# emilk/field_interpolation

Measured on AMD Instinct MI355X. Metric: solved lattice points/sec (assembly+CG to field within 1e-5 of the CPU reference by the solver's estimate: ended at rel. residual 1.1e-08), higher is better.
Workload: dtype f64

## Files before the change

field_interpolation_amd/csrc/fi_assembly.hip:

```cpp

#include "fi_prim.h"

#include "fi_internal.h"
#include "fi_rows.h"
#include "fi_sort.h"
#include "fi_nearest.h"

namespace fi {

namespace {

constexpr int kThreads = 256;

__host__ __device__ inline int packed_index(int i, int j, int nc)
{
	return i * nc - (i * (i - 1)) / 2 + (j - i);
}

template <int NC>
__device__ inline double block_row_sum(const double* B, int q)
{
	double s = 0.0;
#pragma unroll
	for (int j = 0; j < NC; ++j) { s += B[q <= j ? packed_index(q, j, NC) : packed_index(j, q, NC)]; }
// ... 806 lines not shown
		rhs  = c->pending[0]->rhs.as<float>();
	} else {
		key_cat.alloc(sizeof(uint32_t) * total);
		coef_cat.alloc(sizeof(float) * total * NC);
		rhs_cat.alloc(sizeof(float) * total);
		long at = 0;
		for (auto* pb : c->pending) {
			if (pb->nrows == 0) { continue; }
			FI_HIP_TRY(hipMemcpyAsync(key_cat.as<uint32_t>() + at, pb->key.p, sizeof(uint32_t) * pb->nrows,
			                          hipMemcpyDeviceToDevice, st));
			FI_HIP_TRY(hipMemcpyAsync(coef_cat.as<float>() + at * NC, pb->coef.p, sizeof(float) * pb->nrows * NC,
			                          hipMemcpyDeviceToDevice, st));
			FI_HIP_TRY(hipMemcpyAsync(rhs_cat.as<float>() + at, pb->rhs.p, sizeof(float) * pb->nrows,
			                          hipMemcpyDeviceToDevice, st));
			at += pb->nrows;
		}
		key  = key_cat.as<uint32_t>();
		coef = coef_cat.as<float>();
		rhs  = rhs_cat.as<float>();
	}

	DevBuf &row_in = c->scratch[3], &row_sorted = c->scratch[4], &key_sorted = c->scratch[5], &uniq = c->scratch[6],
	       &counts = c->scratch[7], &starts = c->scratch[8], &nruns = c->scratch[9], &tmp = c->scratch[10];
	row_in.alloc(sizeof(uint32_t) * total);
	row_sorted.alloc(sizeof(uint32_t) * total);
	key_sorted.alloc(sizeof(uint32_t) * total);
	uniq.alloc(sizeof(uint32_t) * total);
	counts.alloc(sizeof(uint32_t) * total);
	starts.alloc(sizeof(uint32_t) * total);
	nruns.alloc(sizeof(uint32_t) * 4);
	hipLaunchKernelGGL(k_iota, dim3(blocks_for(total)), dim3(kThreads), 0, st, row_in.as<uint32_t>(), total);
	int end_bit = 1;
	while ((1ull << end_bit) <= invalid) { ++end_bit; }
	size_t tb = 0;
	FI_HIP_TRY(sort_pairs_u32(nullptr, tb, key, key_sorted.as<uint32_t>(), row_in.as<uint32_t>(), row_sorted.as<uint32_t>(),
	                          static_cast<unsigned int>(total), 0, end_bit, st));
	tmp.alloc(tb);
	FI_HIP_TRY(sort_pairs_u32(tmp.p, tb, key, key_sorted.as<uint32_t>(), row_in.as<uint32_t>(), row_sorted.as<uint32_t>(),
	                          static_cast<unsigned int>(total), 0, end_bit, st));
	size_t tb2 = 0;
	FI_HIP_TRY(prim::run_length_encode(nullptr, tb2, key_sorted.as<uint32_t>(), uniq.as<uint32_t>(), counts.as<uint32_t>(),
	                                    nruns.as<uint32_t>(), static_cast<size_t>(total), st));
	DevBuf& tmp2 = c->scratch[11];
	tmp2.alloc(tb2);
	FI_HIP_TRY(prim::run_length_encode(tmp2.p, tb2, key_sorted.as<uint32_t>(), uniq.as<uint32_t>(), counts.as<uint32_t>(),
	                                    nruns.as<uint32_t>(), static_cast<size_t>(total), st));
	DevBuf& tail3 = c->scratch[26];
	tail3.alloc(sizeof(uint32_t) * 3);
	DevBuf& heavy = c->scratch[28];
	heavy.alloc(sizeof(uint32_t) * (static_cast<size_t>(total / kHeavyRows) + 2));
	hipLaunchKernelGGL(k_rle_tail, dim3(1), dim3(1), 0, st, nruns.as<uint32_t>(), uniq.as<uint32_t>(), counts.as<uint32_t>(),
	                   tail3.as<uint32_t>(), heavy.as<uint32_t>());
	uint32_t* h_tail = static_cast<uint32_t*>(pinned(c, 0, 3 * sizeof(uint32_t)));
	FI_HIP_TRY(hipMemcpyAsync(h_tail, tail3.p, 3 * sizeof(uint32_t), hipMemcpyDeviceToHost, st));
// ... 332 lines not shown
```

field_interpolation_amd/csrc/fi_capi.hip:

```cpp
#include "fi_solver_internal.h"
#include "fi_workers.h"
#include "fi_iso.h"
#include "fi_dual.h"
#include "fi_sample.h"
#include "fi_nearest.h"
#include "fi_knn.h"
#include "fi_orient.h"
#include "fi_surface.h"
#include "fi_ray.h"
#include "fi_robust.h"
#include "fi_parts.h"
#include "fi_simplify.h"
#include "fi_smooth.h"
#include "fi_meshpts.h"

#include <memory>

namespace fi {

static thread_local std::string g_error;

void set_error(const char* fmt, ...)
{
	char    buf[1024];
// ... 432 lines not shown
namespace fi {
void finish_assemble_timing(fi_ctx* c)
{
	if (!c->asm_time_pending) { return; }
	c->asm_time_pending = false;
	if (hipEventSynchronize(c->ev_asm1) != hipSuccess) { return; }
	float ms = 0;
	if (hipEventElapsedTime(&ms, c->ev_asm0, c->ev_asm1) == hipSuccess) { c->stats.assemble_ms = ms; }
}
}

int fi_assemble(fi_ctx* c)
{
	FI_API_BEGIN
	fi::check_ctx(c);
	fi::bind_device(c);
	fi::finish_assemble_timing(c);
	if (!c->ev_asm0) {
		FI_HIP_TRY(hipEventCreate(&c->ev_asm0));
		FI_HIP_TRY(hipEventCreate(&c->ev_asm1));
	}
	const hipEvent_t e0 = c->ev_asm0, e1 = c->ev_asm1;
	fi::chain_mark(nullptr);
	FI_HIP_TRY(hipEventRecord(e0, c->stream));
	{
		bool trip = c->generic.ntrip != 0, grad = !fi::holds_value_rows_only(c);
		if (c->facts_forced) {
			trip = c->forced_trip;
			grad = c->forced_grad;
		} else if (c->nranks > 1 && fi::comm_ready(c)) {
			double* slot = (c->scal.as<fi::CgScalars>() + 2)->sums;
			double  v[2] = {trip ? 1.0 : 0.0, grad ? 1.0 : 0.0};
			FI_HIP_TRY(hipMemcpyAsync(slot, v, sizeof(v), hipMemcpyHostToDevice, c->stream));
			fi::allreduce_sum(c, slot, 2);
			FI_HIP_TRY(hipMemcpyAsync(v, slot, sizeof(v), hipMemcpyDeviceToHost, c->stream));
			FI_HIP_TRY(hipStreamSynchronize(c->stream));
			trip = v[0] > 0.0;
			grad = v[1] > 0.0;
		}
		c->any_trip        = trip;
		c->value_rows_only = !grad && !trip;
		c->facts_forced    = false;
	}
	const int reach = fi::model_reach(c->w);
	const int want_reach = reach > 1 ? reach : 1;
	int want_halo = want_reach;
// ... 81 lines not shown
		};
		fi::Worker *helper = nullptr, *helper2 = nullptr;
		try {
			if (!lumped) {
				helper = fi::worker_pool().acquire();
				helper->run(build);
			}
			if (mixed64) {
				helper2 = fi::worker_pool().acquire();
				helper2->run(build2);
			}
		} catch (...) {
		}
		int main_code = FI_OK;
		c->defer_scaling_exchange = true;
		try {
			fi::AllocStream alloc_on(c->stream);
			fi::chain_mark("threads started");
			fi::assemble(c);
			fi::chain_mark("finest: rows assembled");
			fi::generic_assemble(c);
			fi::stencil_prepare(c);
			fi::chain_mark("finest: stencil prepared");
			fi::operator_prepare(c);
			fi::chain_mark("finest: operator prepared");
		} catch (const fi::Fail& f) {
			main_code = f.code;
		} catch (...) {
			main_code = FI_ERR_HIP;
			fi::set_error("unexpected exception while assembling the finest level");
		}
		if (lumped && main_code == FI_OK) {
			try {
				fi::AllocStream alloc_on(c->stream);
				c->twin->defer_scaling_exchange = true;
				fi::twin_assemble_lumped(c);
				fi::chain_mark("finest: lumped replica");
			} catch (const fi::Fail& f) {
				main_code = f.code;
			} catch (...) {
				main_code = FI_ERR_HIP;
				fi::set_error("unexpected exception while building the lumped replica");
			}
		}
		if (helper) {
			helper->wait();
			fi::worker_pool().release(helper);
// ... 359 lines not shown
{
	FI_API_BEGIN
	fi::check_assembled(c);
	fi::bind_device(c);
	FI_REQUIRE(x && y, FI_ERR_INVALID, "null vector");
	c->dtype == FI_F64 ? fi::apply_f64_t<double>(c, x, y) : fi::apply_f64_t<float>(c, x, y);
	FI_API_END
}

int fi_get_Atb_f64(fi_ctx* c, double* out)
{
	FI_API_BEGIN
	fi::check_assembled(c);
	fi::bind_device(c);
	c->dtype == FI_F64 ? fi::get_vec_f64_t<double>(c, c->atb, out) : fi::get_vec_f64_t<float>(c, c->atb, out);
	FI_API_END
}

int fi_get_diag_f64(fi_ctx* c, double* out)
{
	FI_API_BEGIN
	fi::check_assembled(c);
	fi::bind_device(c);
	c->dtype == FI_F64 ? fi::get_vec_f64_t<double>(c, c->diag, out) : fi::get_vec_f64_t<float>(c, c->diag, out);
	FI_API_END
}

int fi_get_stats(const fi_ctx* c, fi_stats* out)
{
	FI_API_BEGIN
	fi::check_ctx(c);
	FI_REQUIRE(out != nullptr, FI_ERR_INVALID, "null output");
	fi::finish_assemble_timing(const_cast<fi_ctx*>(c));
	*out = c->stats;
	out->coarse_unconverged = 0;
	const fi_ctx* top = c->twin && c->twin->coarse ? c->twin : c;
	for (const fi_ctx* l = top->coarse; l; l = l->coarse) {
		if (!l->unwatched_pending || !l->ev_unwatched || !l->pin[2]) { continue; }
		if (hipEventSynchronize(l->ev_unwatched) != hipSuccess) { continue; }
		const fi::CgScalars* was = static_cast<const fi::CgScalars*>(l->pin[2]);
		const bool met = was->done == 1 || was->done == 5 || was->done == 4;
		if (!met) { out->coarse_unconverged += 1; }
		out->coarse_iterations += (met ? was->iter : l->unwatched_expected) - l->unwatched_expected;
	}
	FI_API_END
}

int fi_time_apply(fi_ctx* c, int reps, double* ms_per_launch)
{
	FI_API_BEGIN
	fi::check_assembled(c);
	fi::bind_device(c);
	FI_REQUIRE(reps > 0 && ms_per_launch, FI_ERR_INVALID, "bad arguments");
	fi::ensure_vectors(c);
	fi::CgScalars init{};
	FI_HIP_TRY(hipMemcpyAsync(c->scal.p, &init, sizeof(init), hipMemcpyHostToDevice, c->stream));
	fi::EventPair timer;
	const hipEvent_t e0 = timer.e0, e1 = timer.e1;
	const char* which = fi::tuning_switch("FI_TIME_STEP");
	const int   step = which ? atoi(which) : 0;
	auto launch = [&]() {
		if (step >= 1 && fi::stencil_cheb_available(c)) {
			c->dtype == FI_F64 ? fi::ensure_poly_vectors<double>(c) : fi::ensure_poly_vectors<float>(c);
			if (step == 1) {
				fi::stencil_cheb_step(c, c->r.p, nullptr, c->r.p, c->mg_d.p, 0.3, 0.2, c->partial.as<double>(), 0, 0.0, 0.5);
			} else if (step == 2) {
				fi::stencil_cheb_step(c, c->mg_d.p, c->mg_x.p, c->r.p, c->mg_x.p, 0.3, 0.2, c->partial.as<double>(), 0, 0.5);
			} else {
				fi::stencil_cheb_step(c, c->mg_x.p, c->mg_d.p, c->r.p, c->mg_d.p, 0.3, 0.2, c->partial.as<double>());
			}
		} else {
			fi::apply_AtA(c, c->p.p, c->q.p, c->partial.as<double>());
		}
	};
	launch();
	FI_HIP_TRY(hipEventRecord(e0, c->stream));
	for (int k = 0; k < reps; ++k) { launch(); }
	FI_HIP_TRY(hipEventRecord(e1, c->stream));
	FI_HIP_TRY(hipEventSynchronize(e1));
	float ms = 0;
	FI_HIP_TRY(hipEventElapsedTime(&ms, e0, e1));
	*ms_per_launch = ms / reps;
	FI_API_END
// ... 584 lines not shown
```

field_interpolation_amd/csrc/fi_cg.hip:

```cpp
#include "fi_solver_internal.h"

namespace fi {

namespace {
struct PredKey {
	int    kind, dtype, ndim, gn[3], level, below, mixed, rows_only;
	float  w[8];
	double tol;
	bool operator<(const PredKey& o) const { return std::memcmp(this, &o, sizeof(PredKey)) < 0; }
};
PredKey pred_key(const fi_ctx* c, int kind, double tol)
{
	PredKey k;
	std::memset(&k, 0, sizeof(k));
	k.kind  = kind;
	k.dtype = c->dtype;
	k.ndim  = c->g.ndim;
	for (int d = 0; d < 3; ++d) { k.gn[d] = c->g.gn[d]; }
	k.level = c->level;
	for (const fi_ctx* l = (c->twin && c->twin->coarse ? c->twin->coarse : c->coarse); l; l = l->coarse) { ++k.below; }
	k.mixed     = c->mixed;
	k.rows_only = c->value_rows_only ? 1 : 0;
	const float w[8] = {c->w.data_pos, c->w.data_gradient, c->w.model_0, c->w.model_1, c->w.model_2, c->w.model_3, c->w.model_4,
	                    c->w.gradient_smoothness};
// ... 494 lines not shown
	double  v = mine ? 1.0 : 0.0;
	FI_HIP_TRY(hipMemcpyAsync(flag, &v, sizeof(double), hipMemcpyHostToDevice, c0->stream));
	allreduce_sum(c0, flag, 1);
	FI_HIP_TRY(hipMemcpyAsync(&v, flag, sizeof(double), hipMemcpyDeviceToHost, c0->stream));
	FI_HIP_TRY(hipStreamSynchronize(c0->stream));
	return v > 0.0;
}

bool all_ranks_ok(fi_ctx* c, bool mine)
{
	if (!(c->nranks > 1 && comm_ready(c))) { return mine; }
	double* flag = (c->scal.as<CgScalars>() + 2)->sums + 3;
	double  v = mine ? 0.0 : 1.0;
	FI_HIP_TRY(hipMemcpyAsync(flag, &v, sizeof(double), hipMemcpyHostToDevice, c->stream));
	allreduce_sum(c, flag, 1);
	FI_HIP_TRY(hipMemcpyAsync(&v, flag, sizeof(double), hipMemcpyDeviceToHost, c->stream));
	FI_HIP_TRY(hipStreamSynchronize(c->stream));
	return v == 0.0;
}

template <typename T>
void cg_run(RankSet& R, int max_iterations, float tol)
{
	fi_ctx* c0 = R[0];
	hipStream_t st = c0->stream;
	if (max_iterations <= 0) {
		const int64_t dflt = 2 * static_cast<int64_t>(c0->g.gn[0]) * c0->g.gn[1] * c0->g.gn[2];
		max_iterations = dflt > std::numeric_limits<int>::max() ? std::numeric_limits<int>::max() : static_cast<int>(dflt);
	}
	const double tolerance = tol > 0 ? static_cast<double>(tol) : static_cast<double>(std::numeric_limits<float>::epsilon());

	if (c0->unwatched_pending) {
		c0->unwatched_pending = false;
		FI_HIP_TRY(hipEventSynchronize(c0->ev_unwatched));
		const CgScalars* was = static_cast<const CgScalars*>(pinned(c0, 2, sizeof(CgScalars)));
		const bool as_expected = (was->done == 1 || was->done == 5) && was->iter > 0 && was->iter <= c0->unwatched_expected;
		c0->last_cg_iterations = as_expected ? was->iter : 0;
		c0->pred_recalled[0]   = true;
		c0->cg_count_recalled  = false;
	}
	if (c0->level > 0 && R.size() == 1 && c0->last_cg_iterations == 0) {
		const int n = recall_iterations(c0, 0, tolerance);
		if (n > 0) {
			c0->last_cg_iterations = n;
			c0->last_cg_tol        = tolerance;
			c0->cg_count_recalled  = true;
// ... 323 lines not shown
			FI_HIP_TRY(hipMemcpyAsync(g0.p, c->x.p, elem_size(c) * c->g.nloc, hipMemcpyDeviceToDevice, c->stream));
			kept[i] = &g0;
		}
	}
	cg_run<T>(R, 4000, sizeof(T) == 8 ? 1e-12f : 1e-6f);
	for (size_t i = 0; i < R.size(); ++i) {
		if (kept[i]) { generic_keep_guess_in_empty_tiles(R[i], tile_size, kept[i]->p, R[i]->x.p); }
	}
}

template <typename T>
void tile_pass_t(fi_ctx* c, const float* guess, int tile_size, float* out, int memory)
{
	ensure_vectors(c);
	load_owned<T>(c, c->x, guess, memory);
	RankSet R{c};
	tile_pass_run<T>(R, tile_size);
	store_owned<T>(c, c->x, out, memory);
}

template <typename T>
void jacobi_run(RankSet& R, int sweeps, float weight)
{
	CgScalars init{};
	reset_scalars(R, init);
	for (int s = 0; s < sweeps; ++s) {
		halo_exchange(R, &fi_ctx::x);
		for (fi_ctx* c : R) { apply_AtA(c, c->x.p, c->q.p, nullptr); }
		for (fi_ctx* c : R) {
			const int64_t o = c->g.own_first;
			hipLaunchKernelGGL((k_jacobi_update<T>), dim3(stream_blocks(c->g.nown)), dim3(kThreads), 0, c->stream, c->g.nown,
			                   static_cast<T>(weight), c->atb.as<T>() + o, c->q.as<T>() + o, c->dinv.as<T>() + o,
			                   c->x.as<T>() + o);
		}
	}
	FI_HIP_TRY(hipGetLastError());
}

template <typename T>
void jacobi_t(fi_ctx* c, const float* guess, int sweeps, float weight, float* out, int memory)
{
	ensure_vectors(c);
	load_owned<T>(c, c->x, guess, memory);
	RankSet R{c};
	jacobi_run<T>(R, sweeps, weight);
	store_owned<T>(c, c->x, out, memory);
// ... 114 lines not shown
```

field_interpolation_amd/csrc/fi_internal.h:

```cpp
#pragma once

#include <hip/hip_runtime.h>

#include <chrono>
#include <cstdint>
#include <cstdio>
#include <cstdlib>
#include <string>
#include <utility>
#include <vector>

#include "../../include/fi_hip.h"

namespace fi {

inline const char* test_switch(const char* name) { return getenv(name); }
#ifdef FI_TIMING_BUILD
inline const char* tuning_switch(const char* name) { return getenv(name); }
#else
inline const char* tuning_switch(const char*) { return nullptr; }
#endif

inline std::chrono::steady_clock::time_point& chain_origin()
{
// ... 307 lines not shown
	fi::DevBuf dinv16;
	fi::DevBuf dinv16s;
	bool       dinv16s_valid = false;
	bool       lumped = false;
	fi::DevBuf dlump;
	hipEvent_t ev_asm0 = nullptr, ev_asm1 = nullptr;
	bool       asm_time_pending = false;
	bool       want_lump = false;
	fi::DevBuf lump;
	bool       data_pinned = false;
	double     mg_safe = 4.0;
	int        mg_terms = 5;
	double     mg_pratio = 30.0;
	int        mg_cheb_degree = 0;
	double     mg_cheb_ratio = 0.0;
	int        mg_kcycle = 0;
	fi::DevBuf kc;
	int        mg_smoother = 1;
	bool       any_trip = false;
	bool       facts_forced = false, forced_trip = false, forced_grad = false;
	bool       value_rows_only = false;
	bool       scaling_ghosts = false;
	bool       defer_scaling_exchange = false;
	fi::DevBuf x, r, p, q;
	fi::DevBuf mg_b, mg_x, mg_r, mg_d;
	double     lambda_max = 0;
	int        poly_terms = 0;
	double     poly_ratio = 10.0;
	double     poly_lambda = 0;
	int        last_mg_iterations = 0;
	double     last_mg_tol = 0;
	bool       predictable_start = false;
	double     last_cg_tol = 0;
	bool       unwatched_pending = false;
	int        unwatched_expected = 0;
	hipEvent_t ev_unwatched = nullptr;
	int        last_cg_iterations = 0;
	double     field_tol = 0;
	bool       pred_recalled[2] = {false, false};
	bool       cg_count_recalled = false;
	int        last_outer_iterations = 0;
	int        mg_mode = 0;
	fi::DevBuf partial;
	fi::DevBuf scal;
	fi::CgScalars* scal_host = nullptr;
	void*      pin[3] = {nullptr, nullptr, nullptr};
	size_t     scal_host_cap = 0;
	size_t     pin_bytes[3] = {0, 0, 0};
	int        max_blocks = 0;

	fi::DevBuf scratch[36];

	bool       bx_dot_wanted = false, bx_dot_done = false;
	bool       tail_ok = false;
	fi::DevBuf tail_dia, tail_map, tail_prog;
	bool       tail_prog_valid = false;
	bool       dia_valid = false;
	int        tail_nlev = 0, tail_nops = 0;
	int        tail_lds_floats = 0;

	fi::Comm*  comm = nullptr;
	hipStream_t comm_stream = nullptr;
	hipStream_t level_stream = nullptr;
	hipEvent_t  ev_level = nullptr;
	hipStream_t level_stream2 = nullptr;
	hipStream_t build_stream = nullptr;
	hipEvent_t  ev_build = nullptr;
	hipEvent_t  ev_level2 = nullptr;
	hipEvent_t  ev_ready = nullptr, ev_halo = nullptr;
	fi::DevBuf group_scal;
	bool       owns_stream = true;
	bool       owns_comm = true;
	int        mixed = 0;
	fi_ctx*    twin = nullptr;
	int        tile_ts = 0;
	int        verify_residual = 1;
	fi_stats   stats{};
	std::vector<hipEvent_t> ev;
	std::vector<hipEvent_t> ev_prec;
	int        prec_budget = 0, prec_taken = 0, prec_chain_launches = 0;
	double     prec_chain_bytes = 0;
};

namespace fi {

size_t elem_size(const fi_ctx* c);

void operator_prepare(fi_ctx* c, bool with_scaling = false, const float* lump_in = nullptr);
void apply_AtA(fi_ctx* c, const void* x, void* y, double* pq_partial);
int  apply_num_partials(const fi_ctx* c);
double apply_algorithmic_bytes(const fi_ctx* c);
void error_map(fi_ctx* c, const void* x, void* out);
void exchange_halo(fi_ctx* c, void* v, int width = 0);
void exchange_halo_on(fi_ctx* c, void* v, hipStream_t stream, int width = 0);
bool comm_ready(const fi_ctx* c);
void operator_finish_ghosts(fi_ctx* c);
void operator_rescale_with_ghosts(fi_ctx* c);
void prepare_safe_scaling(fi_ctx* c);

void stencil_prepare(fi_ctx* c);
int  stencil_partials(const fi_ctx* c);
bool stencil_apply(fi_ctx* c, const void* x, void* y, double* partial);
bool stencil_apply_part(fi_ctx* c, const void* x, void* y, double* partial, int part);

bool cells_fused(const fi_ctx* c);
bool stencil_cheb_available(const fi_ctx* c);
int  stencil_cheb_partials(const fi_ctx* c);
void stencil_cheb_step(fi_ctx* c, const void* z, const void* zprev, const void* r, void* znew, double c1, double c2,
                       double* partial, int part = 0, double zprev_scale = 0.0, double pro_scale = 0.0,
                       const unsigned short* scaling = nullptr,
                       int extend = 0,
// ... 50 lines not shown
```

field_interpolation_amd/csrc/fi_levels.hip:

```cpp
#include "fi_solver_internal.h"
#include "fi_workers.h"

namespace fi {

int plan_levels(const fi_ctx* c, int* first_tail)
{
	const int D = c->g.ndim;
	int n[3] = {c->g.gn[0], c->g.gn[1], c->g.gn[2]};
	std::vector<int> lo(c->nranks), hi(c->nranks);
	for (int r = 0; r < c->nranks; ++r) {
		lo[r] = static_cast<int>(static_cast<int64_t>(r) * n[D - 1] / c->nranks);
		hi[r] = static_cast<int>(static_cast<int64_t>(r + 1) * n[D - 1] / c->nranks);
	}
	int levels = 0, tail = 0;
	const bool allow_tail = c->nranks > 1 && !test_switch("FI_NO_REPLICATED_TAIL");
	for (int l = 1; l <= c->levels_wanted; ++l) {
		bool ok = true;
		for (int d = 0; d < D; ++d) {
			n[d] = (n[d] + 1) / 2;
			ok = ok && n[d] >= 8;
		}
		if (!ok) { break; }
		if (c->nranks > 1 && !tail) {
			bool thick = true;
// ... 274 lines not shown
                                                           float* __restrict__ diag)
{
	for (int64_t i = static_cast<int64_t>(blockIdx.x) * kThreads + threadIdx.x; i < n; i += static_cast<int64_t>(gridDim.x) * kThreads) {
		const float v = sums[i];
		const float f = v > 0.0f ? v : 0.0f;
		dlump[i] = f;
		diag[i]  = f;
	}
}

void twin_assemble_lumped(fi_ctx* c)
{
	fi_ctx* t = c->twin;
	t->stream = c->stream;
	for (auto* pb : t->pending) { t->pending_pool.push_back(pb); }
	t->pending.clear();
	generic_clear(t);
	assemble(t);
	const Geom& g = c->g;
	FI_REQUIRE(c->want_lump && c->lump.p, FI_ERR_STATE, "the lumped replica needs the row sums of the fp64 level's assembly");
	generic_assemble(t);
	stencil_prepare(t);
	if (g.nown == g.nloc && t->nranks == 1 && g.nloc > (1 << 16)) {
		operator_prepare(t, true, c->lump.as<float>());
		return;
	}
	t->dlump.alloc(sizeof(float) * g.nloc);
	if (g.nown != g.nloc) { FI_HIP_TRY(hipMemsetAsync(t->dlump.p, 0, sizeof(float) * g.nloc, c->stream)); }
	hipLaunchKernelGGL(k_lumped_diag, dim3(stream_blocks(g.nown)), dim3(kThreads), 0, c->stream, g.nown,
	                   c->lump.as<float>() + g.own_first, t->dlump.as<float>() + g.own_first, t->diag.as<float>() + g.own_first);
	FI_HIP_TRY(hipGetLastError());
	operator_prepare(t, t->nranks == 1);
}

fi_ctx* twin_prepare(fi_ctx* c)
{
	if (c->level != 0) { return nullptr; }
	if (!(c->mixed && c->dtype == FI_F64)) {
		if (c->twin) {
			fi_ctx_destroy(c->twin);
			c->twin = nullptr;
		}
		return nullptr;
	}
	const int D = c->g.ndim;
	{
		long from_points = 0;
// ... 104 lines not shown
```

field_interpolation_amd/csrc/fi_multigrid.hip:

```cpp
#include "fi_solver_internal.h"

namespace fi {

template <typename T>
bool cascade_guess(RankSet& R, RankSet* wide)
{
	bool wrote_wide = false;
	std::vector<RankSet> chains;
	{
		RankSet cur = R;
		for (;;) {
			chains.push_back(cur);
			RankSet next;
			for (fi_ctx* c : cur) {
				if (c->coarse) { next.push_back(c->coarse); }
			}
			if (next.size() != cur.size()) { break; }
			cur = next;
		}
	}
	for (auto& lev : chains) {
		for (fi_ctx* c : lev) { ensure_vectors(c); }
	}
	for (fi_ctx* c : chains.back()) { FI_HIP_TRY(hipMemsetAsync(c->x.p, 0, sizeof(T) * c->g.nloc, c->stream)); }
// ... 437 lines not shown
		}
	} else if (Rfine[0]->nranks > 1) {
		allreduce_sum_vec(Rfine[0], (Rc[0]->*v).p, n, sizeof(T) == 8);
	}
}

RankSet coarse_of(const RankSet& R)
{
	RankSet r;
	for (fi_ctx* c : R) { r.push_back(c->coarse); }
	return r;
}

void apply_all(RankSet& R, Vec in, Vec out, bool partials)
{
	halo_exchange(R, in);
	for (fi_ctx* c : R) { apply_AtA(c, (c->*in).p, (c->*out).p, partials ? c->partial.as<double>() : nullptr); }
}


template <typename T>
void estimate_lambda(RankSet& R)
{
	for (fi_ctx* c : R) { mg_alloc<T>(c); }
	CgScalars init{};
	reset_scalars(R, init);
	auto nbv = [](fi_ctx* c) { return stream_blocks(c->g.nown); };
	for (fi_ctx* c : R) {
		hipLaunchKernelGGL((k_seed<T>), dim3(nbv(c)), dim3(kThreads), 0, c->stream, c->g.nown, global_first(c),
		                   vown<T>(c, &fi_ctx::mg_d));
	}
	const int steps = 10;
	double sums[2] = {0, 0};
	for (int k = 0; k < steps; ++k) {
		apply_all(R, &fi_ctx::mg_d, &fi_ctx::q, false);
		for (fi_ctx* c : R) {
			hipLaunchKernelGGL((k_power_step<T>), dim3(nbv(c)), dim3(kThreads), 0, c->stream, c->g.nown, vown<T>(c, &fi_ctx::q),
			                   vown<T>(c, &fi_ctx::dinv), vown<T>(c, &fi_ctx::mg_d), c->partial.as<double>());
		}
		if (k >= steps - 2) {
			reduce_phase(R, 1, nbv, nbv, -1);
			fi_ctx* c0 = R[0];
			FI_HIP_TRY(hipMemcpyAsync(c0->scal_host, c0->scal.p, sizeof(CgScalars), hipMemcpyDeviceToHost, c0->stream));
			FI_HIP_TRY(hipStreamSynchronize(c0->stream));
			sums[k - (steps - 2)] = c0->scal_host->sums[0];
		}
	}
	const double lambda = (sums[0] > 0 && sums[1] > 0) ? std::sqrt(sums[1] / sums[0]) : 2.0;
	for (fi_ctx* c : R) { c->lambda_max = lambda; }
}

bool smooth_fused_ok(const RankSet& R)
{
	if (test_switch("FI_NO_FUSED_SMOOTHER")) { return false; }
	for (const fi_ctx* c : R) {
		if (!stencil_full_epi_available(c)) { return false; }
	}
	return true;
}
void swap_vectors(RankSet& R, Vec a, Vec b)
{
	if (a == b) { return; }
	for (fi_ctx* c : R) {
		(c->*a).swap(c->*b);
	}
}
template <typename T>
void cheb_smooth_fused(RankSet& R, Vec b, Vec x, int degree, double ratio, bool from_zero)
{
	const double hi = 1.1 * R[0]->lambda_max, lo = hi / ratio;
	const double theta = 0.5 * (hi + lo), delta = 0.5 * (hi - lo), sigma = theta / delta;
	const Vec ring[3] = {x, &fi_ctx::mg_d, &fi_ctx::mg_r};
	int cur = 0, prev = -1;
	auto step = [&](double a, double c1, double c2) {
		const int next = prev < 0 ? (cur + 1) % 3 : 3 - cur - prev;
		halo_exchange(R, ring[cur]);
		for (fi_ctx* c : R) {
			stencil_full_step(c, (c->*ring[cur]).p, prev < 0 ? nullptr : (c->*ring[prev]).p, (c->*b).p, false,
			                  (c->*ring[next]).p, a, c1, c2);
		}
		prev = cur;
		cur  = next;
	};
	bool have_prev = false;
	if (from_zero) {
		for (fi_ctx* c : R) {
			hipLaunchKernelGGL((k_cheb_first16<T>), dim3(stream_blocks(c->g.nown)), dim3(kThreads), 0, c->stream, c->g.nown,
			                   vown<T>(c, b), c->dinv16.as<unsigned short>() + c->g.own_first, vown<T>(c, x),
			                   static_cast<T>(1.0 / theta));
		}
	} else {
		step(1.0, 0.0, 1.0 / theta);
		have_prev = true;
	}
	double rho = 1.0 / sigma;
	for (int k = 1; k < degree; ++k) {
		const double rho_new = 1.0 / (2.0 * sigma - rho);
		const double c1 = rho_new * rho, c2 = 2.0 * rho_new / delta;
		if (!have_prev) { prev = -1; }
		step(1.0 + c1, c1, c2);
		have_prev = true;
		rho = rho_new;
	}
	swap_vectors(R, x, ring[cur]);
}

template <typename T>
void cheb_smooth(RankSet& R, Vec b, Vec x, int degree, double ratio, bool from_zero)
{
	if (smooth_fused_ok(R)) {
		cheb_smooth_fused<T>(R, b, x, degree, ratio, from_zero);
		return;
	}
	const double hi = 1.1 * R[0]->lambda_max, lo = hi / ratio;
	const double theta = 0.5 * (hi + lo), delta = 0.5 * (hi - lo), sigma = theta / delta;
	auto nbv = [](fi_ctx* c) { return stream_blocks(c->g.nown); };
	if (from_zero) {
		for (fi_ctx* c : R) {
			hipLaunchKernelGGL((k_cheb_first<T>), dim3(nbv(c)), dim3(kThreads), 0, c->stream, c->g.nown, vown<T>(c, b),
			                   vown<T>(c, &fi_ctx::dinv), degree > 1 ? vown<T>(c, &fi_ctx::mg_d) : vown<T>(c, x),
			                   static_cast<T>(1.0 / theta));
		}
	} else {
		apply_all(R, x, &fi_ctx::q, false);
		for (fi_ctx* c : R) {
			hipLaunchKernelGGL((k_cheb_init<T>), dim3(nbv(c)), dim3(kThreads), 0, c->stream, c->g.nown, vown<T>(c, b),
			                   vown<T>(c, &fi_ctx::q), vown<T>(c, &fi_ctx::dinv), vown<T>(c, &fi_ctx::mg_r),
			                   vown<T>(c, &fi_ctx::mg_d), vown<T>(c, x), static_cast<T>(1.0 / theta), 0);
		}
	}
	double rho = 1.0 / sigma;
	for (int k = 1; k < degree; ++k) {
// ... 1173 lines not shown
```

field_interpolation_amd/csrc/fi_operator.hip:

```cpp

#include "fi_internal.h"

namespace fi {

namespace {

constexpr int kThreads = 256;

__device__ inline double wave_sum(double v)
{
	for (int o = 32; o > 0; o >>= 1) { v += __shfl_down(v, o, 64); }
	return v;
}

__device__ inline double block_sum(double v)
{
	__shared__ double s[kThreads / 64];
	v = wave_sum(v);
	const int lane = threadIdx.x & 63, wave = threadIdx.x >> 6;
	if (lane == 0) { s[wave] = v; }
	__syncthreads();
	double r = 0;
	if (threadIdx.x == 0) {
		for (int w = 0; w < kThreads / 64; ++w) { r += s[w]; }
// ... 411 lines not shown
	mc.on[5] = w.gradient_smoothness > 0.0f;
	mc.gs    = mc.on[5] ? static_cast<T>(w.gradient_smoothness) : T(0);
	return mc;
}

constexpr int kDiagRows = 4;
template <typename T>
__global__ __launch_bounds__(kThreads) void k_model_diag3(Geom g, ModelCoef<T> mc, T* __restrict__ diag, T* __restrict__ dinv,
                                                          unsigned short* __restrict__ d16, unsigned short* __restrict__ d16s, T factor,
                                                          const float* __restrict__ lump_in, float* __restrict__ dlump_out)
{
	const int ext0 = g.own_hi[0] - g.own_lo[0], ext1 = g.own_hi[1] - g.own_lo[1];
	const int x = static_cast<int>(blockIdx.x) * kThreads + threadIdx.x;
	if (x >= ext0) { return; }
	const int lx = g.own_lo[0] + x, lz = g.own_lo[2] + static_cast<int>(blockIdx.z);
	const int y0 = static_cast<int>(blockIdx.y) * kDiagRows;
	T in[kDiagRows];
#pragma unroll
	for (int j = 0; j < kDiagRows; ++j) {
		const int64_t idx = lx * g.stride[0] + (g.own_lo[1] + y0 + j) * g.stride[1] + lz * g.stride[2];
		if (lump_in) {
			const float v = y0 + j < ext1 ? lump_in[idx] : 0.0f;
			in[j] = static_cast<T>(v > 0.0f ? v : 0.0f);
			if (y0 + j < ext1) { dlump_out[idx] = static_cast<float>(in[j]); }
		} else {
			in[j] = y0 + j < ext1 ? diag[idx] : T(0);
		}
	}
#pragma unroll
	for (int j = 0; j < kDiagRows; ++j) {
		if (y0 + j >= ext1) { break; }
		const int ly = g.own_lo[1] + y0 + j;
		const int64_t idx = lx * g.stride[0] + ly * g.stride[1] + lz * g.stride[2];
		T acc = 0;
#pragma unroll
		for (int d = 0; d < 3; ++d) {
			const int li = d == 0 ? lx : (d == 1 ? ly : lz);
			const int c = li + g.off[d], n = g.gn[d];
			if (mc.on[0]) { acc += mc.w0sq; }
			for (int k = 1; k <= 4; ++k) {
				if (!mc.on[k]) { continue; }
				for (int m = 0; m <= k; ++m) {
					const int a = c - m;
					if (a >= 0 && a + k < n) { acc += mc.c[k][m] * mc.c[k][m]; }
				}
			}
		}
		const T d = in[j] + acc;
		__builtin_nontemporal_store(d, diag + idx);
		if (dinv) {
			const T v = (d != T(0)) ? T(1) / d : T(1);
			__builtin_nontemporal_store(v, dinv + idx);
			__builtin_nontemporal_store(static_cast<unsigned short>(__float_as_uint(static_cast<float>(v)) >> 16), d16 + idx);
		}
		if (d16s) {
			const T dd = d > acc ? d - acc : T(0);
			const T sc = acc + factor * dd;
			const T v  = (sc > T(0)) ? T(1) / sc : T(1);
			__builtin_nontemporal_store(static_cast<unsigned short>(__float_as_uint(static_cast<float>(v)) >> 16), d16s + idx);
		}
	}
}

template <int D, typename T>
void prepare_dim(fi_ctx* c, bool with_scaling, const float* lump_in)
{
	const Geom& g = c->g;
	const ModelCoef<T> mc = make_coef<T>(c->w);
	c->dinv.alloc(sizeof(T) * g.nloc);
	c->dinv16.alloc(sizeof(unsigned short) * g.nloc);
	const bool whole = g.nown == g.nloc;
	const int ext1 = g.own_hi[1] - g.own_lo[1], ext2 = g.own_hi[2] - g.own_lo[2];
	const bool fuse_scaling = with_scaling && whole && c->nranks == 1 && g.nloc > (1 << 16);
	FI_REQUIRE(!lump_in || (D == 3 && !mc.on[5] && ext1 <= 65535 && ext2 <= 65535 && whole && sizeof(T) == 4), FI_ERR_STATE,
	           "lumped replica: unexpected lattice");
	if (D == 3 && !mc.on[5] && ext1 <= 65535 && ext2 <= 65535) {
		if (fuse_scaling) { c->dinv16s.alloc(sizeof(unsigned short) * g.nloc); }
		if (lump_in) { c->dlump.alloc(sizeof(float) * g.nloc); }
		hipLaunchKernelGGL((k_model_diag3<T>), dim3((g.own_hi[0] - g.own_lo[0] + kThreads - 1) / kThreads, (ext1 + kDiagRows - 1) / kDiagRows, ext2),
		                   dim3(kThreads), 0, c->stream, g, mc, c->diag.as<T>(), whole ? c->dinv.as<T>() : static_cast<T*>(nullptr),
		                   whole ? c->dinv16.as<unsigned short>() : static_cast<unsigned short*>(nullptr),
		                   fuse_scaling ? c->dinv16s.as<unsigned short>() : static_cast<unsigned short*>(nullptr),
		                   static_cast<T>(c->lumped ? 1.0 : c->mg_safe), lump_in, lump_in ? c->dlump.as<float>() : static_cast<float*>(nullptr));
		if (fuse_scaling) {
			c->data_pinned   = false;
			c->dinv16s_valid = true;
		}
	} else
	hipLaunchKernelGGL((k_model_diag<D, T>), dim3(blocks_for(g.nown)), dim3(kThreads), 0, c->stream, g, mc,
	                   c->diag.as<T>(), whole ? c->dinv.as<T>() : static_cast<T*>(nullptr),
	                   whole ? c->dinv16.as<unsigned short>() : static_cast<unsigned short*>(nullptr));
	c->scaling_ghosts = false;
	if (!whole) {
		if (c->nranks > 1 && comm_ready(c) && !c->defer_scaling_exchange) {
			exchange_halo(c, c->diag.p, c->min_slab >= c->halo ? c->halo : c->reach);
			c->scaling_ghosts = true;
		}
		hipLaunchKernelGGL((k_invert_diag<T>), dim3(blocks_for(g.nloc)), dim3(kThreads), 0, c->stream, g.nloc,
		                   c->diag.as<T>(), c->dinv.as<T>(), c->dinv16.as<unsigned short>());
	}
	FI_HIP_TRY(hipGetLastError());
}

template <typename T>
void finish_ghosts_t(fi_ctx* c)
{
	const Geom& g = c->g;
	exchange_halo(c, c->diag.p, c->min_slab >= c->halo ? c->halo : c->reach);
	hipLaunchKernelGGL((k_invert_diag<T>), dim3(blocks_for(g.nloc)), dim3(kThreads), 0, c->stream, g.nloc, c->diag.as<T>(),
	                   c->dinv.as<T>(), c->dinv16.as<unsigned short>());
	FI_HIP_TRY(hipGetLastError());
	c->scaling_ghosts = true;
}

template <int D, typename T>
void safe_scaling_dim(fi_ctx* c)
{
	const Geom& g = c->g;
	const ModelCoef<T> mc = make_coef<T>(c->w);
	c->dinv16s.alloc(sizeof(unsigned short) * g.nloc);
	unsigned int* weak = nullptr;
	DevBuf cnt;
	if (g.nloc <= (1 << 16) && c->nranks == 1) {
		cnt.alloc(sizeof(unsigned int));
		FI_HIP_TRY(hipMemsetAsync(cnt.p, 0, sizeof(unsigned int), c->stream));
		weak = cnt.as<unsigned int>();
	}
	hipLaunchKernelGGL((k_safe_scaling<D, T>), dim3(blocks_for(g.nloc)), dim3(kThreads), 0, c->stream, g, mc, c->diag.as<T>(),
	                   static_cast<T>(c->lumped ? 1.0 : c->mg_safe), c->dinv16s.as<unsigned short>(), weak);
	FI_HIP_TRY(hipGetLastError());
	c->data_pinned = false;
	if (weak) {
		unsigned int* h = static_cast<unsigned int*>(pinned(c, 0, sizeof(unsigned int)));
		*h = 1;
		FI_HIP_TRY(hipMemcpyAsync(h, weak, sizeof(unsigned int), hipMemcpyDeviceToHost, c->stream));
		FI_HIP_TRY(hipStreamSynchronize(c->stream));
		c->data_pinned = *h == 0;
	}
	c->dinv16s_valid = true;
}

int cells_partials(const fi_ctx* c) { return capped_blocks(c->cells.ncell); }

template <int D, typename T>
void apply_dim(fi_ctx* c, const T* x, T* y, double* partial)
// ... 225 lines not shown
	c->defer_scaling_exchange = false;
	if (c->nranks <= 1 || !comm_ready(c) || c->g.nown == c->g.nloc) { return; }
	c->dtype == FI_F64 ? finish_ghosts_t<double>(c) : finish_ghosts_t<float>(c);
	c->dinv16s_valid = false;
}

void operator_rescale_with_ghosts(fi_ctx* c)
{
	const Geom& g = c->g;
	if (c->dtype == FI_F64) {
		hipLaunchKernelGGL((k_invert_diag<double>), dim3(blocks_for(g.nloc)), dim3(kThreads), 0, c->stream, g.nloc, c->diag.as<double>(),
		                   c->dinv.as<double>(), c->dinv16.as<unsigned short>());
	} else {
		hipLaunchKernelGGL((k_invert_diag<float>), dim3(blocks_for(g.nloc)), dim3(kThreads), 0, c->stream, g.nloc, c->diag.as<float>(),
		                   c->dinv.as<float>(), c->dinv16.as<unsigned short>());
	}
	FI_HIP_TRY(hipGetLastError());
	c->scaling_ghosts = true;
	c->dinv16s_valid  = false;
}

void prepare_safe_scaling(fi_ctx* c)
{
	const bool f64 = c->dtype == FI_F64;
	switch (c->g.ndim) {
	case 1: f64 ? safe_scaling_dim<1, double>(c) : safe_scaling_dim<1, float>(c); break;
	case 2: f64 ? safe_scaling_dim<2, double>(c) : safe_scaling_dim<2, float>(c); break;
	default: f64 ? safe_scaling_dim<3, double>(c) : safe_scaling_dim<3, float>(c); break;
	}
}

void operator_prepare(fi_ctx* c, bool with_scaling, const float* lump_in)
{
	const bool f64 = c->dtype == FI_F64;
	c->dinv16s_valid = false;
	switch (c->g.ndim) {
	case 1: f64 ? prepare_dim<1, double>(c, with_scaling, lump_in) : prepare_dim<1, float>(c, with_scaling, lump_in); break;
	case 2: f64 ? prepare_dim<2, double>(c, with_scaling, lump_in) : prepare_dim<2, float>(c, with_scaling, lump_in); break;
	default: f64 ? prepare_dim<3, double>(c, with_scaling, lump_in) : prepare_dim<3, float>(c, with_scaling, lump_in); break;
	}
	if (with_scaling && !c->dinv16s_valid) { prepare_safe_scaling(c); }
}

void apply_AtA(fi_ctx* c, const void* x, void* y, double* partial)
{
	const bool f64 = c->dtype == FI_F64;
	switch (c->g.ndim) {
	case 1:
		f64 ? apply_dim<1, double>(c, static_cast<const double*>(x), static_cast<double*>(y), partial)
		    : apply_dim<1, float>(c, static_cast<const float*>(x), static_cast<float*>(y), partial);
		break;
	case 2:
		f64 ? apply_dim<2, double>(c, static_cast<const double*>(x), static_cast<double*>(y), partial)
		    : apply_dim<2, float>(c, static_cast<const float*>(x), static_cast<float*>(y), partial);
		break;
	default:
		f64 ? apply_dim<3, double>(c, static_cast<const double*>(x), static_cast<double*>(y), partial)
		    : apply_dim<3, float>(c, static_cast<const float*>(x), static_cast<float*>(y), partial);
// ... 6 lines not shown
```

field_interpolation_amd/csrc/fi_poly.hip:

```cpp
#include "fi_solver_internal.h"

namespace fi {

bool poly_ok(const fi_ctx* c) { return c->poly_terms > 1 && stencil_cheb_available(c) && c->generic.ntrip == 0 && !c->any_trip && c->tile_ts == 0; }


#ifndef FI_PCG_NT
#define FI_PCG_NT 1
#endif
template <typename T>
__device__ inline void pld16(T* dst, const T* base, int64_t i)
{
	if (FI_PCG_NT) { ld16_nt(dst, base, i); } else { *reinterpret_cast<typename Vec16<T>::V*>(dst) = reinterpret_cast<const typename Vec16<T>::V*>(base)[i]; }
}
template <typename T>
__device__ inline void pst16(T* base, int64_t i, const T* src)
{
	if (FI_PCG_NT) { st16_nt(base, i, src); } else { reinterpret_cast<typename Vec16<T>::V*>(base)[i] = *reinterpret_cast<const typename Vec16<T>::V*>(src); }
}

template <typename T, bool VEC>
__global__ __launch_bounds__(kThreads) void k_pcg_resid(int64_t n, const CgScalars* __restrict__ in, CgScalars* __restrict__ mid,
                                                         int tag, int phase, const double* __restrict__ pq_partial, int pq_count,
                                                         const T* __restrict__ b, const T* __restrict__ q,
// ... 288 lines not shown
				                   static_cast<int>(R.size()), 1, 2);
			} else if (R[0]->nranks > 1) {
				allreduce_sum(R[0], (R[0]->scal.as<CgScalars>() + 2)->sums, 1);
			}
			fi_ctx* c0 = R[0];
			FI_HIP_TRY(hipMemcpyAsync(c0->scal_host, c0->scal.as<CgScalars>() + 2, sizeof(CgScalars), hipMemcpyDeviceToHost, c0->stream));
			FI_HIP_TRY(hipStreamSynchronize(c0->stream));
			sums[k - (steps - 2)] = c0->scal_host->sums[0];
		}
		std::swap(cur, nxt);
	}
	const double lambda = (sums[0] > 0 && sums[1] > 0 && std::isfinite(sums[1])) ? std::sqrt(sums[1] / sums[0]) : 4.0;
	for (fi_ctx* c : R) { c->poly_lambda = lambda; }
	if (sums[0] > 0 && sums[1] > 0 && std::isfinite(sums[1])) {
		std::lock_guard<std::mutex> lock(g_lambda_mutex);
		if (g_lambda_cache.size() > 4096) { g_lambda_cache.clear(); }
		g_lambda_cache[lambda_key(R[0])] = lambda;
	}
}

template <typename T>
void cg_run_poly(RankSet& R, int max_iterations, float tol)
{
	fi_ctx* c0 = R[0];
	hipStream_t st = c0->stream;
	const int terms = c0->poly_terms;
	if (max_iterations <= 0) {
		const int64_t dflt = 2 * static_cast<int64_t>(c0->g.gn[0]) * c0->g.gn[1] * c0->g.gn[2];
		max_iterations = dflt > std::numeric_limits<int>::max() ? std::numeric_limits<int>::max() : static_cast<int>(dflt);
	}
	const double tolerance = tol > 0 ? static_cast<double>(tol) : static_cast<double>(std::numeric_limits<float>::epsilon());
	for (fi_ctx* c : R) { ensure_poly_vectors<T>(c); }
	if (!(c0->poly_lambda > 0)) { estimate_poly_lambda<T>(R); }

	EventPair timer;
	const hipEvent_t e0 = timer.e0, e1 = timer.e1;
	FI_HIP_TRY(hipEventRecord(e0, st));

	double lam_scale = 1.0;
	if (const char* env = test_switch("FI_POLY_LAMBDA_SCALE")) { lam_scale = atof(env) > 0 ? atof(env) : 1.0; }
	double theta = 1.0, delta = 1.0;
	std::vector<double> c1s, c2s;
	auto set_interval = [&]() {
		const double lam = (c0->poly_lambda > 1.0 ? c0->poly_lambda : 1.0) * lam_scale;
		const double hi = 1.1 * lam, lo = hi / (c0->poly_ratio > 1.0 ? c0->poly_ratio : 10.0);
		theta = 0.5 * (hi + lo);
// ... 381 lines not shown
	__syncthreads();
	if (sh_quit) { return; }
	const T alpha = static_cast<T>(sh_alpha), beta = static_cast<T>(sh_beta);
	double acc = 0.0;
	for (int64_t i = static_cast<int64_t>(blockIdx.x) * kThreads + threadIdx.x; i < n;
	     i += static_cast<int64_t>(gridDim.x) * kThreads) {
		const T pv = first ? z[i] : z[i] + beta * p[i];
		const T sv = first ? w[i] : w[i] + beta * s[i];
		p[i] = pv;
		s[i] = sv;
		x[i] += alpha * pv;
		const T rv = r[i] - alpha * sv;
		r[i] = rv;
		acc += static_cast<double>(rv) * static_cast<double>(rv);
	}
	double accv[1] = {acc}, sum[1];
	block_sum<1>(accv, sum);
	if (threadIdx.x == 0) { prr[blockIdx.x] = sum[0]; }
}

template <typename T>
void cg_run_poly_sr(RankSet& R, int max_iterations, float tol)
{
	fi_ctx* c0 = R[0];
	hipStream_t st = c0->stream;
	const int terms = c0->poly_terms;
	if (max_iterations <= 0) {
		const int64_t dflt = 2 * static_cast<int64_t>(c0->g.gn[0]) * c0->g.gn[1] * c0->g.gn[2];
		max_iterations = dflt > std::numeric_limits<int>::max() ? std::numeric_limits<int>::max() : static_cast<int>(dflt);
	}
	const double tolerance = tol > 0 ? static_cast<double>(tol) : static_cast<double>(std::numeric_limits<float>::epsilon());
	for (fi_ctx* c : R) {
		ensure_poly_vectors<T>(c);
		const size_t bytes = sizeof(T) * c->g.nloc;
		if (c->mg_r.bytes < bytes) {
			c->mg_r.alloc(bytes);
			FI_HIP_TRY(hipMemsetAsync(c->mg_r.p, 0, bytes, c->stream));
		}
	}
	if (!(c0->poly_lambda > 0)) { estimate_poly_lambda<T>(R); }
	EventPair timer;
	const hipEvent_t e0 = timer.e0, e1 = timer.e1;
	FI_HIP_TRY(hipEventRecord(e0, st));

	double lam_scale = 1.0;
	if (const char* env = test_switch("FI_POLY_LAMBDA_SCALE")) { lam_scale = atof(env) > 0 ? atof(env) : 1.0; }
// ... 210 lines not shown
```

Measured before the change: 1.840 billion.

## Defer diagonal scaling preparation until a solver needs it; cache iota buffer

Operator preparation (diagonal, inverse diagonal and 16-bit scaling) for the finest level in mixed-precision runs, and for the lumped replica, is now deferred. A light pass forms only the smoother scaling, and the remaining outputs are built lazily by ensure_scaling, called at every solver or diag entry point. The iota index buffer used by the row sort is kept across calls instead of being relaunched each time, and the weak-count buffer is kept on the context. This trims kernels from assembly, at the cost of extra lazy-initialisation state that every consumer must remember to trigger.

Result: faster. 1.863 billion (median of 6 runs) (+1.2%).

```diff
diff --git a/field_interpolation_amd/csrc/fi_assembly.hip b/field_interpolation_amd/csrc/fi_assembly.hip
--- a/field_interpolation_amd/csrc/fi_assembly.hip
+++ b/field_interpolation_amd/csrc/fi_assembly.hip
@@ -852,6 +852,7 @@
 
 	DevBuf &row_in = c->scratch[3], &row_sorted = c->scratch[4], &key_sorted = c->scratch[5], &uniq = c->scratch[6],
 	       &counts = c->scratch[7], &starts = c->scratch[8], &nruns = c->scratch[9], &tmp = c->scratch[10];
+	if (row_in.bytes < sizeof(uint32_t) * total) { c->iota_n = 0; }
 	row_in.alloc(sizeof(uint32_t) * total);
 	row_sorted.alloc(sizeof(uint32_t) * total);
 	key_sorted.alloc(sizeof(uint32_t) * total);
@@ -859,7 +860,10 @@
 	counts.alloc(sizeof(uint32_t) * total);
 	starts.alloc(sizeof(uint32_t) * total);
 	nruns.alloc(sizeof(uint32_t) * 4);
-	hipLaunchKernelGGL(k_iota, dim3(blocks_for(total)), dim3(kThreads), 0, st, row_in.as<uint32_t>(), total);
+	if (c->iota_n < total) {
+		hipLaunchKernelGGL(k_iota, dim3(blocks_for(total)), dim3(kThreads), 0, st, row_in.as<uint32_t>(), total);
+		c->iota_n = total;
+	}
 	int end_bit = 1;
 	while ((1ull << end_bit) <= invalid) { ++end_bit; }
 	size_t tb = 0;
diff --git a/field_interpolation_amd/csrc/fi_capi.hip b/field_interpolation_amd/csrc/fi_capi.hip
--- a/field_interpolation_amd/csrc/fi_capi.hip
+++ b/field_interpolation_amd/csrc/fi_capi.hip
@@ -478,6 +478,7 @@
 	}
 	const hipEvent_t e0 = c->ev_asm0, e1 = c->ev_asm1;
 	fi::chain_mark(nullptr);
+	c->scaling_deferred = false;
 	FI_HIP_TRY(hipEventRecord(e0, c->stream));
 	{
 		bool trip = c->generic.ntrip != 0, grad = !fi::holds_value_rows_only(c);
@@ -605,7 +606,7 @@
 			fi::generic_assemble(c);
 			fi::stencil_prepare(c);
 			fi::chain_mark("finest: stencil prepared");
-			fi::operator_prepare(c);
+			if (!(mixed64 && c->twin && fi::operator_defer(c))) { fi::operator_prepare(c); }
 			fi::chain_mark("finest: operator prepared");
 		} catch (const fi::Fail& f) {
 			main_code = f.code;
@@ -1011,6 +1012,7 @@
 	FI_API_BEGIN
 	fi::check_assembled(c);
 	fi::bind_device(c);
+	fi::ensure_scaling(c);
 	c->dtype == FI_F64 ? fi::get_vec_f64_t<double>(c, c->diag, out) : fi::get_vec_f64_t<float>(c, c->diag, out);
 	FI_API_END
 }
@@ -1048,6 +1050,7 @@
 	const hipEvent_t e0 = timer.e0, e1 = timer.e1;
 	const char* which = fi::tuning_switch("FI_TIME_STEP");
 	const int   step = which ? atoi(which) : 0;
+	if (step >= 1) { fi::ensure_scaling(c); }
 	auto launch = [&]() {
 		if (step >= 1 && fi::stencil_cheb_available(c)) {
 			c->dtype == FI_F64 ? fi::ensure_poly_vectors<double>(c) : fi::ensure_poly_vectors<float>(c);
diff --git a/field_interpolation_amd/csrc/fi_cg.hip b/field_interpolation_amd/csrc/fi_cg.hip
--- a/field_interpolation_amd/csrc/fi_cg.hip
+++ b/field_interpolation_amd/csrc/fi_cg.hip
@@ -540,6 +540,7 @@
 template <typename T>
 void cg_run(RankSet& R, int max_iterations, float tol)
 {
+	for (fi_ctx* c : R) { ensure_scaling(c); }
 	fi_ctx* c0 = R[0];
 	hipStream_t st = c0->stream;
 	if (max_iterations <= 0) {
@@ -909,6 +910,7 @@
 template <typename T>
 void jacobi_run(RankSet& R, int sweeps, float weight)
 {
+	for (fi_ctx* c : R) { ensure_scaling(c); }
 	CgScalars init{};
 	reset_scalars(R, init);
 	for (int s = 0; s < sweeps; ++s) {
diff --git a/field_interpolation_amd/csrc/fi_internal.h b/field_interpolation_amd/csrc/fi_internal.h
--- a/field_interpolation_amd/csrc/fi_internal.h
+++ b/field_interpolation_amd/csrc/fi_internal.h
@@ -353,6 +353,7 @@
 	bool       value_rows_only = false;
 	bool       scaling_ghosts = false;
 	bool       defer_scaling_exchange = false;
+	bool       scaling_deferred = false;
 	fi::DevBuf x, r, p, q;
 	fi::DevBuf mg_b, mg_x, mg_r, mg_d;
 	double     lambda_max = 0;
@@ -381,6 +382,8 @@
 	int        max_blocks = 0;
 
 	fi::DevBuf scratch[36];
+	int64_t    iota_n = 0;
+	fi::DevBuf weak_cnt;
 
 	bool       bx_dot_wanted = false, bx_dot_done = false;
 	bool       tail_ok = false;
@@ -418,6 +421,8 @@
 size_t elem_size(const fi_ctx* c);
 
 void operator_prepare(fi_ctx* c, bool with_scaling = false, const float* lump_in = nullptr);
+bool operator_defer(fi_ctx* c, const float* lump_in = nullptr);
+void ensure_scaling(fi_ctx* c);
 void apply_AtA(fi_ctx* c, const void* x, void* y, double* pq_partial);
 int  apply_num_partials(const fi_ctx* c);
 double apply_algorithmic_bytes(const fi_ctx* c);
diff --git a/field_interpolation_amd/csrc/fi_levels.hip b/field_interpolation_amd/csrc/fi_levels.hip
--- a/field_interpolation_amd/csrc/fi_levels.hip
+++ b/field_interpolation_amd/csrc/fi_levels.hip
@@ -320,7 +320,7 @@
 	generic_assemble(t);
 	stencil_prepare(t);
 	if (g.nown == g.nloc && t->nranks == 1 && g.nloc > (1 << 16)) {
-		operator_prepare(t, true, c->lump.as<float>());
+		if (!operator_defer(t, c->lump.as<float>())) { operator_prepare(t, true, c->lump.as<float>()); }
 		return;
 	}
 	t->dlump.alloc(sizeof(float) * g.nloc);
diff --git a/field_interpolation_amd/csrc/fi_multigrid.hip b/field_interpolation_amd/csrc/fi_multigrid.hip
--- a/field_interpolation_amd/csrc/fi_multigrid.hip
+++ b/field_interpolation_amd/csrc/fi_multigrid.hip
@@ -483,6 +483,7 @@
 template <typename T>
 void estimate_lambda(RankSet& R)
 {
+	for (fi_ctx* c : R) { ensure_scaling(c); }
 	for (fi_ctx* c : R) { mg_alloc<T>(c); }
 	CgScalars init{};
 	reset_scalars(R, init);
@@ -529,6 +530,7 @@
 template <typename T>
 void cheb_smooth_fused(RankSet& R, Vec b, Vec x, int degree, double ratio, bool from_zero)
 {
+	for (fi_ctx* c : R) { ensure_scaling(c); }
 	const double hi = 1.1 * R[0]->lambda_max, lo = hi / ratio;
 	const double theta = 0.5 * (hi + lo), delta = 0.5 * (hi - lo), sigma = theta / delta;
 	const Vec ring[3] = {x, &fi_ctx::mg_d, &fi_ctx::mg_r};
@@ -569,6 +571,7 @@
 template <typename T>
 void cheb_smooth(RankSet& R, Vec b, Vec x, int degree, double ratio, bool from_zero)
 {
+	for (fi_ctx* c : R) { ensure_scaling(c); }
 	if (smooth_fused_ok(R)) {
 		cheb_smooth_fused<T>(R, b, x, degree, ratio, from_zero);
 		return;
diff --git a/field_interpolation_amd/csrc/fi_operator.hip b/field_interpolation_amd/csrc/fi_operator.hip
--- a/field_interpolation_amd/csrc/fi_operator.hip
+++ b/field_interpolation_amd/csrc/fi_operator.hip
@@ -457,7 +457,7 @@
 		if (lump_in) {
 			const float v = y0 + j < ext1 ? lump_in[idx] : 0.0f;
 			in[j] = static_cast<T>(v > 0.0f ? v : 0.0f);
-			if (y0 + j < ext1) { dlump_out[idx] = static_cast<float>(in[j]); }
+			if (dlump_out && y0 + j < ext1) { dlump_out[idx] = static_cast<float>(in[j]); }
 		} else {
 			in[j] = y0 + j < ext1 ? diag[idx] : T(0);
 		}
@@ -482,7 +482,7 @@
 			}
 		}
 		const T d = in[j] + acc;
-		__builtin_nontemporal_store(d, diag + idx);
+		if (diag) { __builtin_nontemporal_store(d, diag + idx); }
 		if (dinv) {
 			const T v = (d != T(0)) ? T(1) / d : T(1);
 			__builtin_nontemporal_store(v, dinv + idx);
@@ -497,10 +497,12 @@
 	}
 }
 
+enum { kPrepFull = 0, kPrepLight = 1, kPrepLate = 2 };
 template <int D, typename T>
-void prepare_dim(fi_ctx* c, bool with_scaling, const float* lump_in)
+void prepare_dim(fi_ctx* c, bool with_scaling, const float* lump_in, int mode = kPrepFull)
 {
 	const Geom& g = c->g;
+	const bool light = mode == kPrepLight, late = mode == kPrepLate;
 	const ModelCoef<T> mc = make_coef<T>(c->w);
 	c->dinv.alloc(sizeof(T) * g.nloc);
 	c->dinv16.alloc(sizeof(unsigned short) * g.nloc);
@@ -509,14 +511,17 @@
 	const bool fuse_scaling = with_scaling && whole && c->nranks == 1 && g.nloc > (1 << 16);
 	FI_REQUIRE(!lump_in || (D == 3 && !mc.on[5] && ext1 <= 65535 && ext2 <= 65535 && whole && sizeof(T) == 4), FI_ERR_STATE,
 	           "lumped replica: unexpected lattice");
+	FI_REQUIRE(mode == kPrepFull || (lump_in && (late || fuse_scaling)), FI_ERR_STATE, "lumped replica: no light pass on this lattice");
 	if (D == 3 && !mc.on[5] && ext1 <= 65535 && ext2 <= 65535) {
 		if (fuse_scaling) { c->dinv16s.alloc(sizeof(unsigned short) * g.nloc); }
 		if (lump_in) { c->dlump.alloc(sizeof(float) * g.nloc); }
 		hipLaunchKernelGGL((k_model_diag3<T>), dim3((g.own_hi[0] - g.own_lo[0] + kThreads - 1) / kThreads, (ext1 + kDiagRows - 1) / kDiagRows, ext2),
-		                   dim3(kThreads), 0, c->stream, g, mc, c->diag.as<T>(), whole ? c->dinv.as<T>() : static_cast<T*>(nullptr),
-		                   whole ? c->dinv16.as<unsigned short>() : static_cast<unsigned short*>(nullptr),
+		                   dim3(kThreads), 0, c->stream, g, mc, light ? static_cast<T*>(nullptr) : c->diag.as<T>(),
+		                   whole && !light ? c->dinv.as<T>() : static_cast<T*>(nullptr),
+		                   whole && !light ? c->dinv16.as<unsigned short>() : static_cast<unsigned short*>(nullptr),
 		                   fuse_scaling ? c->dinv16s.as<unsigned short>() : static_cast<unsigned short*>(nullptr),
-		                   static_cast<T>(c->lumped ? 1.0 : c->mg_safe), lump_in, lump_in ? c->dlump.as<float>() : static_cast<float*>(nullptr));
+		                   static_cast<T>(c->lumped ? 1.0 : c->mg_safe), lump_in,
+		                   lump_in && !late ? c->dlump.as<float>() : static_cast<float*>(nullptr));
 		if (fuse_scaling) {
 			c->data_pinned   = false;
 			c->dinv16s_valid = true;
@@ -555,7 +560,7 @@
 	const ModelCoef<T> mc = make_coef<T>(c->w);
 	c->dinv16s.alloc(sizeof(unsigned short) * g.nloc);
 	unsigned int* weak = nullptr;
-	DevBuf cnt;
+	DevBuf& cnt = c->weak_cnt;
 	if (g.nloc <= (1 << 16) && c->nranks == 1) {
 		cnt.alloc(sizeof(unsigned int));
 		FI_HIP_TRY(hipMemsetAsync(cnt.p, 0, sizeof(unsigned int), c->stream));
@@ -827,6 +832,7 @@
 
 void prepare_safe_scaling(fi_ctx* c)
 {
+	ensure_scaling(c);
 	const bool f64 = c->dtype == FI_F64;
 	switch (c->g.ndim) {
 	case 1: f64 ? safe_scaling_dim<1, double>(c) : safe_scaling_dim<1, float>(c); break;
@@ -835,10 +841,41 @@
 	}
 }
 
+bool operator_defer(fi_ctx* c, const float* lump_in)
+{
+	const Geom& g = c->g;
+	if (test_switch("FI_EAGER_SCALING") || c->nranks != 1 || g.nown != g.nloc) { return false; }
+	if (lump_in) {
+		if (!(c->lumped && c->dtype == FI_F32 && g.ndim == 3 && g.nloc > (1 << 16))) { return false; }
+		c->dinv16s_valid = false;
+		prepare_dim<3, float>(c, true, lump_in, kPrepLight);
+		FI_REQUIRE(c->dinv16s_valid, FI_ERR_STATE, "lumped replica: the light pass did not form the smoother's scaling");
+	} else {
+		c->dinv.alloc(elem_size(c) * g.nloc);
+		c->dinv16.alloc(sizeof(unsigned short) * g.nloc);
+		c->dinv16s_valid = false;
+	}
+	c->scaling_ghosts   = false;
+	c->scaling_deferred = true;
+	return true;
+}
+
+void ensure_scaling(fi_ctx* c)
+{
+	if (!c->scaling_deferred) { return; }
+	if (c->lumped) {
+		c->scaling_deferred = false;
+		prepare_dim<3, float>(c, false, c->dlump.as<float>(), kPrepLate);
+		return;
+	}
+	operator_prepare(c);
+}
+
 void operator_prepare(fi_ctx* c, bool with_scaling, const float* lump_in)
 {
 	const bool f64 = c->dtype == FI_F64;
 	c->dinv16s_valid = false;
+	c->scaling_deferred = false;
 	switch (c->g.ndim) {
 	case 1: f64 ? prepare_dim<1, double>(c, with_scaling, lump_in) : prepare_dim<1, float>(c, with_scaling, lump_in); break;
 	case 2: f64 ? prepare_dim<2, double>(c, with_scaling, lump_in) : prepare_dim<2, float>(c, with_scaling, lump_in); break;
diff --git a/field_interpolation_amd/csrc/fi_poly.hip b/field_interpolation_amd/csrc/fi_poly.hip
--- a/field_interpolation_amd/csrc/fi_poly.hip
+++ b/field_interpolation_amd/csrc/fi_poly.hip
@@ -334,6 +334,7 @@
 template <typename T>
 void cg_run_poly(RankSet& R, int max_iterations, float tol)
 {
+	for (fi_ctx* c : R) { ensure_scaling(c); }
 	fi_ctx* c0 = R[0];
 	hipStream_t st = c0->stream;
 	const int terms = c0->poly_terms;
@@ -761,6 +762,7 @@
 template <typename T>
 void cg_run_poly_sr(RankSet& R, int max_iterations, float tol)
 {
+	for (fi_ctx* c : R) { ensure_scaling(c); }
 	fi_ctx* c0 = R[0];
 	hipStream_t st = c0->stream;
 	const int terms = c0->poly_terms;
```
